# orm011/mplan2vdl

Measured on AMD Instinct MI355X. Metric: rows/s, TPC-H Q6 SF100 (fused VDL scan), + achieved HBM GB/s in roofline, higher is better.
Workload: dtype int64; 1 GPU; tpch_q6_sf100; rows_total=600037902, rows_per_gpu=600037902, bytes_per_row=28, finalise=local

## Files before the change

mplan2vdl_amd/csrc/vdl_jit.cpp:

```cpp
#include "vdl_jit.h"

#include <dlfcn.h>
#include <fcntl.h>
#include <sys/stat.h>
#include <unistd.h>

#include <atomic>
#include <cerrno>
#include <cstdio>
#include <cstdlib>
#include <cstring>
#include <fstream>
#include <map>
#include <mutex>
#include <sstream>

namespace vdl {
namespace jit {

namespace {

#ifndef VDL_PROJ_U
#define VDL_PROJ_U 4
#endif
// ... 223 lines not shown
        const MAggDesc &a = D.agg[j];
        o << "    d.agg[" << j << "].kind = " << a.kind << "; d.agg[" << j << "].used = " << a.used << "u; d.agg[" << j << "].plain = " << a.plain << "u; d.agg[" << j
          << "].constant = " << lit(a.constant) << ";\n";
        for (int k = 0; k < C.ncol; k++)
            if ((a.used >> k) & 1u) o << "    d.agg[" << j << "].fa[" << k << "] = " << lit(a.fa[k]) << "; d.agg[" << j << "].fs[" << k << "] = " << lit(a.fs[k]) << ";\n";
    }
    if (kind != MSCAN) {
        o << "    d.take = " << D.take << "u; d.nout = " << D.nout << "; d.bitmap_only = " << D.bitmap_only << "; d.carry = " << D.carry << "u;\n";
        for (int k = 0; k < D.nout; k++) o << "    d.out_col[" << k << "] = " << D.out_col[k] << ";\n";
        o << "    d.nexpr = " << D.nexpr << ";\n";
        for (int k = 0; k < D.nexpr; k++) o << "    d.expr_at[" << k << "] = " << D.expr_at[k] << "; d.expr_len[" << k << "] = " << D.expr_len[k] << ";\n";
    }
    o << "    return d;\n}\n}  // namespace vdl\n";
    return o.str();
}

static bool has_sat_diff(const MsArgs &C, const MScanDesc &D) {
    for (int k = 0; k < C.ncol; k++) if (D.dkind[k] == VC_SUBS) return true;
    return false;
}

static bool has_lookup_decode(const MsArgs &C) { return (C.decode & C.derived) != 0; }

std::string scan_source(Kind kind, const MsArgs &C, const MScanDesc &D, const Shape &sh) {
    std::ostringstream o;
    o << "#define VDL_SPEC_UNROLL _Pragma(\"unroll\")\n";
    const bool rt = sh.rt_bounds;
    if (rt) o << "#define VDL_RT_BOUNDS 1\n";
    if (has_sat_diff(C, D)) o << "#define VDL_SAT_DIFF 1\n";
    if (has_lookup_decode(C)) o << "#define VDL_LOOKUP_DECODE 1\n";
    if (kind == MSCAN && sh.batch) o << "#define VDL_BATCH " << sh.batch << "\n#define VDL_BATCH_NAGG " << D.nagg << "\n";
    if (kind == MSCAN && sh.census) o << "#define VDL_CENSUS 1\n";
    if (kind == MSCAN && C.packed) o << "#define VDL_PACKED 1\n";
    if (kind == MSCAN && C.lazy && C.packed) {
        auto ulit = [](int64_t x) { return std::to_string((uint64_t)x & 0xffffffffull) + "u"; };
        o << "#define VDL_STAGED_PRE";
        for (int c = 0; c < C.ncol; c++) {
            if (!((C.filtered >> c) & 1u) || ((C.lazy >> c) & 1u)) continue;
            if (rt) o << rt_filter_line(C, D, c, (C.packed >> c) & 1u);
            else if ((C.packed >> c) & 1u)
                o << " _Pragma(\"unroll\") for (int r = 0; r < RW; r++) alive[r] = alive[r] & ((uint32_t)v[" << c << "][r] >= " << ulit(D.flo[c]) << ") & ((uint32_t)v[" << c
                  << "][r] <= " << ulit(D.fhi[c]) << ");";
            else
                o << " _Pragma(\"unroll\") for (int r = 0; r < RW; r++) alive[r] = alive[r] & (v[" << c << "][r] >= " << lit(D.flo[c]) << ") & (v[" << c << "][r] <= "
                  << lit(D.fhi[c]) << ");";
        }
        o << "\n#define VDL_STAGED_POST";
        for (int c = 0; c < C.ncol; c++) {
            if (!((C.lazy >> c) & 1u)) continue;
            const int w = C.width(c);
            o << " { const __amdgpu_buffer_rsrc_t rs_ = buf_rsrc((const char *)Cr.ptr[" << c << "] + tile0 * " << w << ", (uint32_t)(tile_rows * " << w
              << ")); _Pragma(\"unroll\") for (int r = 0; r < RW; r++) {";
            if (sh.census)
                o << " { const uint64_t m_ = __ballot(pass[r]); const uint64_t a_ = (uint64_t)Cr.ptr[" << c << "] + (uint64_t)(rowid[r] - Cr.row0) * " << w << "ull;"
                  << " const int ln_ = (int)(threadIdx.x & 63u); int lo_ = ln_ - (int)((a_ & 127ull) / " << w << "ull); if (lo_ < 0) lo_ = 0;"
                  << " const bool first_ = pass[r] && ((m_ >> lo_) & ((1ull << (ln_ - lo_)) - 1ull)) == 0ull;"
                  << " const uint64_t f_ = __ballot(first_); if (ln_ == 0) census_cnt[" << c << "] += (unsigned long long)__popcll(f_); }";
            o << " v[" << c << "][r] = buf_load_one<" << w << ">(rs_, pass[r], (uint32_t)(rowid[r] - Cr.row0 - tile0) * " << w << "u); } }";
        }
        o << "\n";
    } else if (kind == MSCAN && C.lazy && C.queued) {
        o << "#define VDL_QUEUE_FILTER";
        for (int c = 0; c < C.ncol; c++)
            if (!((C.derived >> c) & 1u) && !((C.lazy >> c) & 1u) && ((C.filtered >> c) & 1u) && rt) o << rt_filter_line(C, D, c, false);
            else if (!((C.derived >> c) & 1u) && !((C.lazy >> c) & 1u) && ((C.filtered >> c) & 1u))
                o << " _Pragma(\"unroll\") for (int r = 0; r < RW; r++) alive[r] = alive[r] & (v[" << c << "][r] >= " << lit(D.flo[c]) << ") & (v[" << c << "][r] <= " << lit(D.fhi[c]) << ");";
// ... 24 lines not shown
                l << " if (RW % 2 == 0) { _Pragma(\"unroll\") for (int r = 0; r < RW; r += 2) { const int r1 = r + 1 < RW ? r + 1 : r; v[" << c << "][r] = 0; v[" << c
                  << "][r1] = 0;" << census(c, w, (std::string(mask) + "[r] | " + mask + "[r1]").c_str()) << " if (" << mask << "[r] | " << mask << "[r1]) { const int64_t i0 = rowid[r] - Cr.row0; if (i0 + 1 < Cr.n) { const " << vt << " x = *(const " << vt
                  << " *)((const char *)Cr.ptr[" << c << "] + i0 * " << w << "); v[" << c << "][r] = x.x; v[" << c << "][r1] = x.y; } else if (" << mask << "[r]) v[" << c
                  << "][r] = load_scalar(Cr.ptr[" << c << "], " << w << ", i0); } } } else {";
            }
            l << " _Pragma(\"unroll\") for (int r = 0; r < RW; r++) { v[" << c << "][r] = 0; if (" << mask << "[r]) v[" << c << "][r] = load_scalar(Cr.ptr[" << c << "], "
              << w << ", rowid[r] - Cr.row0); }";
            if (pairs) l << " }";
            return l.str();
        };
        o << "#define VDL_STAGED_PRE";
        for (int st = 0; st <= 3; st++)
            for (int c = 0; c < C.ncol; c++) {
                if (((C.derived >> c) & 1u) || C.stage(c) != st) continue;
                if (st > 0) o << load(c, "alive");
                if (((C.filtered >> c) & 1u) && rt) o << rt_filter_line(C, D, c, false);
                else if ((C.filtered >> c) & 1u)
                    o << " _Pragma(\"unroll\") for (int r = 0; r < RW; r++) alive[r] = alive[r] & (v[" << c << "][r] >= " << lit(D.flo[c]) << ") & (v[" << c << "][r] <= "
                      << lit(D.fhi[c]) << ");";
            }
        for (int c = 0; c < C.ncol; c++) if (!((C.derived >> c) & 1u) && C.stage(c) == 14) o << load(c, "alive");
        o << "\n#define VDL_STAGED_POST";
        for (int c = 0; c < C.ncol; c++) if (!((C.derived >> c) & 1u) && C.stage(c) == 15) o << load(c, "pass");
        o << "\n";
    }
    o << "#define VDL_PROJ_U " << VDL_PROJ_U_HOST << "\n" << kEmbedded << "\n" << desc_text(kind, C, D, "", rt);
    const char *b = sh.vec ? "true" : "false";
    if (kind == MSCAN && sh.batch)
        o << "extern \"C\" __global__ __launch_bounds__(256) void " << entry_name(kind, C, D, sh) << "(const vdl::MsArgs Cr, const vdl::MsBatch B) {\n"
             "    constexpr vdl::MsArgs C = vdl::jit_args();\n"
             "    constexpr vdl::MScanDesc D = vdl::jit_desc();\n"
             "    vdl::mscan_body<" << sh.nc << ", " << sh.u << ", " << b << ", " << b << ", " << (sh.grouped ? "true" : "false") << ", false, false>(C, Cr, D, *B.d[0], B);\n}\n";
    else if (kind == MSCAN)
        o << "extern \"C\" __global__ __launch_bounds__(256) void " << entry_name(kind, C, D, sh) << "(const vdl::MsArgs Cr, const vdl::MScanDesc *__restrict__ Dp) {\n"
             "    constexpr vdl::MsArgs C = vdl::jit_args();\n"
             "    constexpr vdl::MScanDesc D = vdl::jit_desc();\n"
             "    vdl::mscan_body<" << sh.nc << ", " << sh.u << ", " << b << ", " << b << ", " << (sh.grouped ? "true" : "false") << ", " << (sh.der ? "true" : "false")
          << ", " << (C.lazy ? "true" : "false") << ">(C, Cr, D, *Dp);\n}\n";
    else if (kind == SELECT)
        o << "extern \"C\" __global__ __launch_bounds__(256) void " << entry_name(kind) << "(const vdl::MsArgs Cr, const vdl::MScanDesc *__restrict__ Dp) {\n"
             "    constexpr vdl::MsArgs C = vdl::jit_args();\n"
             "    constexpr vdl::MScanDesc D = vdl::jit_desc();\n"
             "    vdl::project_select_body<" << sh.nc << ", vdl::kProjU, " << b << ", " << b << ">(C, Cr, D, *Dp);\n}\n";
    else
        o << "extern \"C\" __global__ __launch_bounds__(256) void " << entry_name(kind) << "(const vdl::MsArgs Cr, const vdl::MScanDesc *__restrict__ Dp, const uint16_t *__restrict__ scratch,\n"
             "        const int64_t *__restrict__ counts, const int64_t *__restrict__ offsets) {\n"
             "    constexpr vdl::MsArgs C = vdl::jit_args();\n"
             "    constexpr vdl::MScanDesc D = vdl::jit_desc();\n"
             "    vdl::project_take_body<" << sh.nc << ">(C, Cr, D, *Dp, scratch, counts, offsets);\n}\n";
    return o.str();
}
std::string mscan_source(const MsArgs &C, const MScanDesc &D, const Shape &sh) { return scan_source(MSCAN, C, D, sh); }
std::string front_source(const MsArgs &Cs, const MScanDesc &Ds, const MsArgs &Ct, const MScanDesc &Dt, const Shape &sh, int nct) {
    std::ostringstream o;
    o << "#define VDL_SPEC_UNROLL _Pragma(\"unroll\")\n";
    if (sh.rt_bounds) o << "#define VDL_RT_BOUNDS 1\n";
    if (has_sat_diff(Cs, Ds) || has_sat_diff(Ct, Dt)) o << "#define VDL_SAT_DIFF 1\n";
    if (has_lookup_decode(Cs) || has_lookup_decode(Ct)) o << "#define VDL_LOOKUP_DECODE 1\n";
    o << "#define VDL_PROJ_U " << VDL_PROJ_U_HOST << "\n#define VDL_FRONT_BATCH " << VDL_FRONT_BATCH_HOST << "\n" << kEmbedded << "\n" << desc_text(SELECT, Cs, Ds, "_s", sh.rt_bounds) << desc_text(TAKE, Ct, Dt, "_t", sh.rt_bounds);
    const char *b = sh.vec ? "true" : "false";
    o << "extern \"C\" __global__ __launch_bounds__(256) void " << entry_name(FRONT) << "(const vdl::MsArgs Csr, const vdl::MScanDesc *__restrict__ Dsp, const vdl::MsArgs Ctr,\n"
         "        const vdl::MScanDesc *__restrict__ Dtp, const vdl::FrontLook lk) {\n"
         "    constexpr vdl::MsArgs Cs = vdl::jit_args_s();\n"
         "    constexpr vdl::MScanDesc Ds = vdl::jit_desc_s();\n"
         "    constexpr vdl::MsArgs Ct = vdl::jit_args_t();\n"
         "    constexpr vdl::MScanDesc Dt = vdl::jit_desc_t();\n"
         "    vdl::project_front_body<" << sh.nc << ", " << nct << ", vdl::kProjU, " << b << ", " << b << ">(Cs, Csr, Ds, *Dsp, Ct, Ctr, Dt, *Dtp, lk);\n}\n";
    return o.str();
}
const char *entry_name(Kind kind) { return kind == MSCAN ? "vdl_jit_mscan" : kind == SELECT ? "vdl_jit_project_select" : kind == FRONT ? "vdl_jit_project_front" : "vdl_jit_project_take"; }
std::string entry_name(Kind kind, const MsArgs &C, const MScanDesc &D, const Shape &sh) {
    if (kind != MSCAN) return entry_name(kind);
    char tag[16];
    snprintf(tag, sizeof tag, "%06llx", (unsigned long long)(fnv(desc_text(kind, C, D, "", sh.rt_bounds)) & 0xffffffull));
    int eager_filters = 0;
    for (int c = 0; c < C.ncol; c++) eager_filters += ((C.filtered >> c) & 1u) && !((C.derived >> c) & 1u) && C.stage(c) == 0;
    return std::string("vdl_jit_mscan_") + (sh.grouped ? "grouped_" : "") + (C.packed ? "packed_" : "") + "u" + std::to_string(sh.u) + (C.lazy ? "_staged" + std::to_string(eager_filters) + "_" : "_") +
           (sh.census ? "census_" : "") + tag + (sh.batch ? "_batch" + std::to_string(sh.batch) : "") + (sh.rt_bounds ? "_rtb" : "");
}

bool compile(const std::string &src, const std::string &arch, std::vector<char> &code, std::string &log, Origin *origin) {
    if (origin) *origin = COMPILED;
    std::string key = std::to_string(fnv(src)) + "_" + std::to_string(src.size()) + "_" + arch;
    {
        Rtc &r0 = rtc();
        int major = 0, minor = 0;
        if (r0.lib && r0.version && r0.version(&major, &minor) == 0) key += "_rtc" + std::to_string(major) + "." + std::to_string(minor);
    }
    {
        std::lock_guard<std::mutex> g(g_mu);
        auto it = g_code.find(key);
        if (it != g_code.end()) { code = it->second; g_from_memory++; if (origin) *origin = FROM_MEMORY; return true; }
    }
    if (const char *dump = getenv("VDL_JIT_DUMP")) {
        std::ofstream f(std::string(dump) + "/vdl_" + key + ".hip");
        f << src;
    }
    const std::string dir = trusted_cache_dir();
    std::string path;
    if (!dir.empty()) {
        path = dir + "/vdl_" + key + ".vdlco";
        if (cache_read(path, src, code)) { std::lock_guard<std::mutex> g(g_mu); g_code[key] = code; g_from_disk++; if (origin) *origin = FROM_DISK; return true; }
    }
    Rtc &r = rtc();
    if (!r.lib || !r.why.empty()) { log = r.why.empty() ? "libhiprtc not usable" : r.why; return false; }
    void *prog = nullptr;
    if (r.create(&prog, src.c_str(), "vdl_jit_scan.hip", 0, nullptr, nullptr) != 0) { log = "hiprtcCreateProgram failed"; return false; }
    const std::string a = "--offload-arch=" + arch;
    const char *opts[] = {a.c_str(), "-O3", "-std=c++17"};
    const int rc = r.compile(prog, 3, opts);
// ... 30 lines not shown
```

mplan2vdl_amd/csrc/vdl_mscan_body.h:

```cpp
#pragma once
#include "vdl_scan_desc.h"
#include "vdl_front_index.h"

#ifndef VDL_SPEC_UNROLL
#define VDL_SPEC_UNROLL
#endif

namespace vdl {

typedef long long ll2 __attribute__((ext_vector_type(2)));
typedef int i32x2 __attribute__((ext_vector_type(2)));
typedef short i16x2 __attribute__((ext_vector_type(2)));
typedef char i8x2 __attribute__((ext_vector_type(2)));

template <int N> struct IntTag { static constexpr int value = N; };

namespace {


constexpr int kWave = 64;
constexpr int kMsBlock = 256;
#ifndef VDL_PROJ_U
#define VDL_PROJ_U 4
#endif
// ... 740 lines not shown
            int64_t t[RW];
            eval_term<NC, RW>(d, v, rowid, t);
            if (GROUPED) {
                if (rk == R_SUM) {
#pragma unroll
                    for (int r = 0; r < RW; r++) atomicAdd((unsigned long long *)&mytab[off[r] + 1 + j], (unsigned long long)t[r]);
                } else if (rk == R_MAX) {
#pragma unroll
                    for (int r = 0; r < RW; r++) atomicMax((long long *)&mytab[off[r] + 1 + j], (long long)t[r]);
                } else {
#pragma unroll
                    for (int r = 0; r < RW; r++) atomicMin((long long *)&mytab[off[r] + 1 + j], (long long)t[r]);
                }
            } else {
                int64_t s = r_identity(rk);
                if (rk == R_SUM) {
#pragma unroll
                    for (int r = 0; r < RW; r++) s = (int64_t)((uint64_t)s + (uint64_t)(pass[r] ? t[r] : 0));
                } else if (rk == R_MIN) {
#pragma unroll
                    for (int r = 0; r < RW; r++) s = (pass[r] && t[r] < s) ? t[r] : s;
                } else {
#pragma unroll
                    for (int r = 0; r < RW; r++) s = (pass[r] && t[r] > s) ? t[r] : s;
                }
                int64_t *slot = &lds[(int64_t)j * BS + tid];
                *slot = r_combine(rk, *slot, s);
            }
        }
    };

    const int64_t ntiles = Cr.n / TILE;
#ifdef VDL_PACKED
    if (!GROUPED && !DER && C.packed) {
        static_assert(32 % ROWS == 0, "a lane's 32 values of a stripe split into row slices");
        const int lane = tid & (kWave - 1);
        const int wave = __builtin_amdgcn_readfirstlane(tid / kWave);
        const int64_t nstripes = (Cr.n + 2047) / 2048, wstride = (int64_t)gridDim.x * (BS / kWave);
        for (int64_t s = (int64_t)blockIdx.x * (BS / kWave) + wave; s < nstripes; s += wstride) {
            uint32_t pw[NC][32];
#pragma unroll
            for (int c = 0; c < NC; c++) {
                if ((C.packed >> c) & 1u) {
                    const int b = C.bits(c);
                    const char *p = (const char *)Cr.ptr[c] + ((s * b) * kWave + lane) * 4;
#pragma unroll
                    for (int k = 0; k < 32; k++)
                        if (k < b) pw[c][k] = stream_load<NT, uint32_t>(p + (int64_t)k * (kWave * 4));
                }
            }
            __builtin_amdgcn_sched_barrier(0);
            const int64_t tile0 = s * 2048, tile_rows = Cr.n - tile0 < 2048 ? Cr.n - tile0 : 2048;
#pragma unroll
            for (int j0 = 0; j0 < 32; j0 += ROWS) {
                int64_t v[NC][ROWS], rowid[ROWS];
#pragma unroll
                for (int r = 0; r < ROWS; r++) rowid[r] = Cr.row0 + tile0 + (int64_t)(j0 + r) * kWave + lane;
#pragma unroll
                for (int c = 0; c < NC; c++) {
                    if ((C.packed >> c) & 1u) {
#pragma unroll
                        for (int r = 0; r < ROWS; r++) v[c][r] = (int64_t)unpack_bits(pw[c], j0 + r, C.bits(c));
                    } else if (c < C.ncol && !((C.lazy >> c) & 1u)) {
#pragma unroll
                        for (int r = 0; r < ROWS; r++) {
                            const int64_t i = rowid[r] - Cr.row0;
// ... 492 lines not shown
```

mplan2vdl_amd/csrc/vdl_scan_desc.h:

```cpp
#pragma once
#if defined(__HIPCC_RTC__)
typedef signed char int8_t;
typedef short int16_t;
typedef int int32_t;
typedef long long int64_t;
typedef unsigned char uint8_t;
typedef unsigned short uint16_t;
typedef unsigned int uint32_t;
typedef unsigned long long uint64_t;
typedef unsigned long long uintptr_t;
#define INT64_MAX 0x7fffffffffffffffLL
#define INT64_MIN (-INT64_MAX - 1)
#else
#include <cstdint>
#endif

#if defined(__HIPCC__) || defined(__HIPCC_RTC__)
#define VDL_SD __host__ __device__
#else
#define VDL_SD
#endif

namespace vdl {

// ... 88 lines not shown
    int64_t key_mask = 0;
    KeyComp comp[kMaxKeyComps];
    MAggDesc agg[kMaxGroupAggs];
    KeyStep key[kMaxKeySteps];
    unsigned long long *census = nullptr;
    uint32_t carry = 0;
    int64_t out_cap = INT64_MAX;
};
constexpr int kMaxCarry = 2;

constexpr int kMaxBatch = 8;
constexpr int kMaxBatchWords = 32;
constexpr int kMaxBatchGrouped = 4;
constexpr int kGroupLdsWords = 8192;
struct MsBatch {
    const MScanDesc *d[kMaxBatch] = {};
    int64_t *partials = nullptr;
};

struct MsArgs {
    int ncol = 0;
    uint32_t steps = 0;
    uint64_t widths = 0;
    uint32_t filtered = 0;
    uint32_t derived = 0;
    uint32_t lazy = 0;
    uint32_t decode = 0;
    uint64_t stages = 0;
    VDL_SD constexpr int stage(int c) const { return (int)((stages >> (4 * c)) & 15u); }
    int queued = 0;
    uint32_t packed = 0;
    uint64_t pbits = 0;
    VDL_SD constexpr int bits(int c) const { return c < 10 ? (int)((pbits >> (6 * c)) & 63u) : 0; }
    int64_t n = 0, row0 = 0;
    int64_t rowid_base = 0;
    const void *ptr[kMaxVCols] = {};
    VDL_SD constexpr int width(int c) const { return (int)((widths >> (4 * c)) & 15u); }
};

}
```

mplan2vdl_amd/csrc/vdl_scan_form.h:

```cpp
#pragma once
#include "vdl_scan_desc.h"

namespace vdl {

struct ScanForm {
    enum Kind { EAGER, STAGED, QUEUE, PACKED } kind = EAGER;
    static constexpr int kAllFilters = kMaxVCols;
    int eager_filters = 0;
    bool every_column = false;
    int u = 0;

    static ScanForm from_code(int code, int u = 0) {
        ScanForm f;
        f.u = u;
        f.kind = code <= 0 ? EAGER : code == 3 ? QUEUE : code >= 5 ? PACKED : STAGED;
        if (f.kind == STAGED) f.eager_filters = code == 4 ? kAllFilters : code;
        f.every_column = code >= 6;
        return f;
    }
    const char *suffix() const {
        return kind == EAGER ? "" : kind == QUEUE ? ",queue" : kind == PACKED ? (every_column ? ",packed" : ",packed,late")
             : eager_filters == kAllFilters ? ",lateall" : eager_filters > 1 ? ",late2" : ",late";
    }
};

}
```

mplan2vdl_amd/csrc/vdl_specialise.cpp:

```cpp
#include "vdl_specialise.h"

namespace vdl {
namespace eng {

void count_build(vdl_plan *p, const std::string &role, jit::Origin from) {
    std::pair<int, int> &b = p->jit_builds[role];
    b.first++;
    b.second += from != jit::COMPILED;
}
std::string builds_text(const vdl_plan *p, const std::string &role) {
    const auto it = p->jit_builds.find(role);
    if (it == p->jit_builds.end()) return "";
    return "from cache: " + std::to_string(it->second.second) + " of " + std::to_string(it->second.first) + " builds of " + role + "; ";
}

static jit::Shape jit_shape(const MScanCols &cols, const ScanLaunch &cfg, const ScanForm &f, bool rt) {
    jit::Shape sh;
    sh.rt_bounds = rt;
    mscan_variant_shape(cfg, &sh.nc, &sh.u, &sh.vec, &sh.grouped, &sh.der);
    sh.nc = cols.ncol;
    for (int k = 0; k < cols.ncol; k++) sh.der |= cols.kind[k] != VC_DIRECT;
    const char *u = getenv(sh.grouped ? "VDL_JIT_GROUP_U" : "VDL_JIT_U");
    if (u && atoi(u) >= 1 && atoi(u) <= 8) sh.u = atoi(u);
    if (f.u > 0) sh.u = f.u;
    else if (f.kind == ScanForm::PACKED) sh.u = getenv("VDL_JIT_U") ? atoi(getenv("VDL_JIT_U")) : 2;
    return sh;
}
static std::string jit_name(const jit::Shape &sh, const MScanCols &cols) {
    return "k_mscan_specialised<" + std::to_string(sh.nc) + "," + std::to_string(sh.u) + "," + (sh.vec ? "vec" : "novec") + "," + (sh.grouped ? "grouped" : "global") +
           (sh.der ? ",derived" : "") + (cols.image ? ",img" : "") + (cols.limage ? ",limg" : "") + ">";
}
static ScanForm form_asked_for() { return getenv("VDL_JIT_LATE") ? ScanForm::from_code(std::max(1, atoi(getenv("VDL_JIT_LATE")))) : ScanForm{}; }

static const std::vector<ScanColumn> &scan_columns(const vdl_plan *p, size_t s) {
    const size_t ns = p->fused.scans.size();
    return s < ns ? p->fused.scans[s].cols : p->fused.gscans[s - ns].cols;
}
static std::string short_name(const std::string &name) { return name.substr(name.find('.') == std::string::npos ? 0 : name.find('.') + 1); }
static std::string stages_text(const vdl_plan *p, size_t s, const MsArgs &args) {
    const std::vector<ScanColumn> &sc = scan_columns(p, s);
    std::string o;
    for (int k = 0; k < args.ncol && k < (int)sc.size(); k++) {
        const int st = args.stage(k);
        if (!st) continue;
        o += (o.empty() ? "" : " ") + short_name(sc[(size_t)k].name) + "@" + (st == 15 ? std::string("last") : st == 14 ? std::string("lookups") : std::to_string(st));
    }
    return o;
}
static std::string packed_text(const vdl_plan *p, size_t s, const MScanCols &cols) {
    const std::vector<ScanColumn> &sc = scan_columns(p, s);
    std::string o;
    for (int k = 0; k < cols.ncol && (size_t)k < sc.size(); k++)
        if ((cols.packed >> k) & 1u) o += (o.empty() ? "" : " ") + short_name(sc[(size_t)k].name) + ":" + std::to_string(cols.pbits[k]);
    return o;
}
static double sampled_selectivity(vdl_ctx *c, const void *dev, int width, int64_t n, int64_t lo, int64_t hi) {
    if (const char *a = getenv("VDL_JIT_ASSUME_SELECTIVITY")) return atof(a);
    if (n <= 0 || !dev || c->device < 0) return 1.0;
    const int64_t chunk = std::min<int64_t>(4096, n), pieces = std::max<int64_t>(1, std::min<int64_t>(16, n / chunk));
    std::vector<char> host((size_t)(chunk * width));
    int64_t in = 0, seen = 0;
    for (int64_t k = 0; k < pieces; k++) {
        const int64_t at = pieces > 1 ? (n - chunk) / (pieces - 1) * k : 0;
// ... 67 lines not shown
            }
            if (eager != 1) { why = "the queue form wants exactly one filter column with the tile"; return false; }
            args.queued = 1;
            args.stages = 0;
        }
        return true;
    }
    if (grouped || s >= p->fused.scans.size()) { why = "the packed form serves global aggregate scans only, not grouped scans"; return false; }
    const ScanPlan &sp = p->fused.scans[s];
    for (const ScanColumn &sc : sp.cols)
        if (sc.kind != VC_DIRECT) { why = "the packed form serves scans over table columns only, not scans with derived columns"; return false; }
    if (!c->images) { why = "column images are off"; return false; }
    if (u != 1 && u != 2 && u != 4 && u != 8 && u != 16) { why = "the packed form takes 1, 2, 4, 8 or 16 row pairs per slice (a lane's 32 values of a stripe split evenly)"; return false; }
    out.own_cols = std::make_shared<MScanCols>();
    out.own_desc = std::make_shared<MScanDesc>();
    MScanCols &pc = *out.own_cols;
    MScanDesc &pd = *out.own_desc;
    int64_t bpr = 0;
    bind_mscan(c, sp, pc, pd, &bpr, p->row_offset, f.every_column ? 2 : 1);
    pd.block_partials = d.block_partials;
    out.cols = &pc;
    out.desc = &pd;
    if (pc.ncol > 10) { why = "the packed form takes at most 10 columns"; return false; }
    if (!pc.packed) { why = f.every_column ? "no column has a packed image the scan may read" : "no filter column has a packed image the scan may read"; return false; }
    out.args = mscan_args(pc);
    if (!f.every_column) {
        MsArgs &args = out.args;
        uint32_t used = 0;
        for (int j = 0; j < pd.nagg; j++) if (pd.agg[j].kind != AGG_FIRST) used |= pd.agg[j].used;
        for (int k = 0; k < pc.ncol; k++)
            if (!((pc.packed >> k) & 1u) && !pc.filtered[k] && ((used >> k) & 1u)) { args.stages |= (uint64_t)15 << (4 * k); args.lazy |= 1u << k; }
        if (!args.lazy) { why = "no column to read late"; return false; }
    }
    return true;
}

struct Specialised {
    std::shared_ptr<jit::Kernel> k;
    int grid = 0, per_cu = 0;
    ScanForm form;
    size_t code_bytes = 0;
    std::string name, stages, packed;
    BoundForm b;
};
static bool build_specialised(vdl_ctx *c, vdl_plan *p, size_t s, bool grouped, const ScanForm &f, const MScanCols &cols, const MScanDesc &d, Specialised &out, std::string &why,
                              bool census = false) {
    out = Specialised{};
    jit::Shape sh = jit_shape(cols, p->mcfg[s], f, p->jit_rt_bounds);
    sh.census = census;
    std::vector<char> code;
    if (!bind_form(c, p, s, grouped, f, sh.u, cols, d, out.b, why)) return false;
    const MsArgs &args = out.b.args;
    const MScanDesc &desc = *out.b.desc;
    jit::Origin from = jit::COMPILED;
    if (!jit::compile(jit::mscan_source(args, desc, sh), c->arch, code, why, &from)) { why = why.substr(0, 400); return false; }
    count_build(p, "scan " + std::to_string(s), from);
    if (code.size() > (size_t)96 << 10) { why = "the descriptor did not fold (" + std::to_string(code.size()) + " B of code)"; return false; }
    out.k = jit::load(code, why, jit::entry_name(jit::MSCAN, args, desc, sh));
    if (!out.k) return false;
    int per_cu = 0;
    if (hipModuleOccupancyMaxActiveBlocksPerMultiprocessor(&per_cu, out.k->fn, 256, mscan_lds_bytes(desc, grouped)) != hipSuccess || per_cu < 1) {
        (void)hipGetLastError();
        per_cu = 2;
    }
    if (per_cu > 8) per_cu = 8;
    const int64_t tile = (int64_t)256 * 2 * sh.u;
    int64_t grid = (int64_t)c->num_cus * per_cu;
    const int64_t most = f.kind == ScanForm::PACKED ? (img::stripes(out.b.cols->n) + 3) / 4 : out.b.cols->n / tile;
    if (grid > most) grid = most;
    if (grid < 1) grid = 1;
    out.grid = (int)grid; out.per_cu = per_cu; out.code_bytes = code.size(); out.form = f; out.form.u = sh.u;
    out.name = jit_name(sh, *out.b.cols);
    out.name.insert(out.name.size() - 1, std::string(f.suffix()) + (sh.rt_bounds ? ",rtb" : ""));
    out.stages = stages_text(p, s, args);
    out.packed = packed_text(p, s, *out.b.cols);
    return true;
}
static std::string form_text(const Specialised &sp) {
    return (sp.packed.empty() ? "" : ", packed: " + sp.packed) + (sp.stages.empty() ? "" : ", read late: " + sp.stages);
}
static void install_form(vdl_plan *p, size_t s, const Specialised &sp) {
    int64_t *parts = p->mdesc[s].block_partials;
    p->mcols[s] = *sp.b.cols;
    p->mdesc[s] = *sp.b.desc;
    p->mdesc[s].block_partials = parts;
    p->mcfg[s].grid = sp.grid;
    p->mjit[s] = sp.k;
    p->mjit_form[s] = sp.form;
}
bool specialise_scan(vdl_ctx *c, vdl_plan *p, size_t s, bool grouped, std::string *kname) {
    Specialised sp;
    std::string why;
    const ScanForm late = form_asked_for();
    std::string why_late;
    if (late.kind != ScanForm::EAGER && !build_specialised(c, p, s, grouped, late, p->mcols[s], p->mdesc[s], sp, why_late) && late.kind == ScanForm::PACKED)
        p->jit_note += "scan " + std::to_string(s) + ": no packed form (" + why_late + "); ";
    if (!sp.k && !build_specialised(c, p, s, grouped, ScanForm{}, p->mcols[s], p->mdesc[s], sp, why)) { p->jit_note += "scan " + std::to_string(s) + ": not specialised (" + why + "); "; return false; }
    install_form(p, s, sp);
    *kname = sp.name;
    p->jit_note += "scan " + std::to_string(s) + ": " + sp.name + ", " + std::to_string(sp.code_bytes) + " B of code, " + std::to_string(sp.per_cu) + " blocks/CU" + form_text(sp) + "; " +
                   builds_text(p, "scan " + std::to_string(s));
    return true;
}

struct TimingEvents {
// ... 7 lines not shown
        HIP_CHECK(hipEventRecord(ev.a, c->stream));
        launch();
        HIP_CHECK(hipEventRecord(ev.b, c->stream));
        HIP_CHECK(hipEventSynchronize(ev.b));
        float t = 0;
        HIP_CHECK(hipEventElapsedTime(&t, ev.a, ev.b));
        if (rep > 0) times.push_back(t);
    }
    std::sort(times.begin(), times.end());
    return times[times.size() / 2];
}

void tune_specialised(vdl_ctx *c, vdl_plan *p, int64_t *dev_words) {
    const size_t ns = p->fused.scans.size(), ng = p->fused.gscans.size();
    TimingEvents ev;
    HIP_CHECK(hipEventCreate(&ev.a));
    HIP_CHECK(hipEventCreate(&ev.b));
    auto median_ms = [&](auto &&launch) { return median_launch_ms(c, ev, launch); };
    for (size_t s = 0; s < ns + ng; s++) {
        if (!p->mjit[s]) continue;
        const bool grouped = s >= ns;
        int64_t *out = dev_words + (grouped ? p->gword_offset[s - ns] : p->word_offset[s]);
        Specialised best;
        float best_ms = 0;
        std::string tried;
        std::vector<std::pair<int, int>> cands = {{2, 0}, {3, 0}, {4, 0}, {6, 0}, {0, 1}, {3, 1}, {2, 1}, {1, 1}, {3, 2}, {2, 2}, {4, 2}, {4, 3}, {3, 3}, {6, 3},
                                                  {2, 4}, {3, 4}, {4, 4}};
        int pin_u = 0, pin_late = -1;
        if (const char *pin = getenv("VDL_JIT_PIN")) {
            if (const char *q = strstr(pin, "u=")) pin_u = atoi(q + 2);
            if (const char *q = strstr(pin, "late=")) pin_late = atoi(q + 5);
            if (pin_u > 0) cands = {{pin_u, std::max(pin_late, 0)}};
        }
        std::vector<std::pair<int, int>> packed_forms = {{2, 5}, {4, 5}, {8, 5}, {16, 5}, {2, 6}, {4, 6}, {8, 6}};
        const char *packed_env = getenv("VDL_JIT_PACKED");
        if (pin_u > 0 || (packed_env && strcmp(packed_env, "0") == 0)) packed_forms.clear();
        else if (packed_env && strcmp(packed_env, "only") == 0) cands.clear();
        if (!packed_forms.empty()) {
            BoundForm b;
            std::string why;
            if (!bind_form(c, p, s, grouped, ScanForm::from_code(5), 2, p->mcols[s], p->mdesc[s], b, why) &&
                !bind_form(c, p, s, grouped, ScanForm::from_code(6), 2, p->mcols[s], p->mdesc[s], b, why)) packed_forms.clear();
        }
        cands.insert(cands.end(), packed_forms.begin(), packed_forms.end());
        const MScanCols *cols = &p->mcols[s];
        const MScanDesc *desc = &p->mdesc[s];
        MScanCols plain_cols;
        std::unique_ptr<MScanDesc> plain_desc;
        if (p->mjit_form[s].kind == ScanForm::PACKED) {
            plain_desc = std::make_unique<MScanDesc>();
            int64_t bpr = 0;
            bind_mscan(c, p->fused.scans[s], plain_cols, *plain_desc, &bpr, p->row_offset);
            plain_desc->block_partials = p->mdesc[s].block_partials;
            cols = &plain_cols;
            desc = plain_desc.get();
        }
        int best_u = 0;
        for (auto &cu : cands) {
            const ScanForm f = ScanForm::from_code(cu.second, cu.first ? cu.first : best_u);
            if (f.u <= 0 || (f.kind != ScanForm::PACKED && (int64_t)256 * 2 * f.u > cols->n)) continue;
            if (f.kind == ScanForm::STAGED && f.eager_filters == 1 && cu.first == best_u) continue;
            Specialised cand;
            std::string why;
            if (!build_specialised(c, p, s, grouped, f, *cols, *desc, cand, why)) continue;
            ScanLaunch cfg = p->mcfg[s];
            cfg.grid = cand.grid;
            HIP_CHECK(hipMemcpyAsync(p->mdev[s]->p, cand.b.desc, sizeof(MScanDesc), hipMemcpyHostToDevice, c->stream));
            const float ms = median_ms([&] { HIP_CHECK(launch_mscan(*cand.b.cols, *cand.b.desc, (const MScanDesc *)p->mdev[s]->p, cfg, grouped, false, out, false, c->stream, cand.k->fn)); });
            tried += " u=" + std::to_string(f.u) + f.suffix() + ":" + std::to_string((int)(ms * 1000)) + "us";
            if (!best.k || ms < best_ms * 0.98f) { best = cand; best_ms = ms; }
            if (f.kind == ScanForm::EAGER && (best_u == 0 || cand.k == best.k)) best_u = f.u;
        }
        if (!best.k) continue;
        if (!grouped && use_kscan(p->fused.scans[s]) && p->block_partials[s] && pin_u <= 0) {
            const float ms = median_ms([&] {
                HIP_CHECK(launch_scan(p->sargs[s], p->scfg[s], c->stream));
                HIP_CHECK(launch_scan_finish(p->sargs[s].block_partials, p->scfg[s].grid, p->sargs[s].nagg, nullptr, p->sargs[s], out, c->stream));
            });
            tried += std::string(" k_scan:") + std::to_string((int)(ms * 1000)) + "us";
            if (ms < best_ms * 0.98f) {
                p->kscan[s] = 1;
                p->mjit[s] = nullptr;
                p->jit_note += "scan " + std::to_string(s) + " tuned:" + tried + " -> " + scan_kernel_name(p->scfg[s]) + "; " + builds_text(p, "scan " + std::to_string(s));
                if ((int)s == p->dominant) p->dominant_kernel = std::string(scan_kernel_name(p->scfg[s])) + "_grid" + std::to_string(p->scfg[s].grid);
                continue;
            }
        }
        install_form(p, s, best);
        p->jit_note += "scan " + std::to_string(s) + " tuned:" + tried + " -> " + best.name + (best.packed.empty() ? "" : " (packed: " + best.packed + ")") +
                       (best.stages.empty() ? "" : " (read late: " + best.stages + ")") + "; " + builds_text(p, "scan " + std::to_string(s));
        if ((int)s == p->dominant)
            p->dominant_kernel = best.name + "_grid" + std::to_string(best.grid) + (grouped ? "_rep" + std::to_string(p->mdesc[s].replicas) : "");
    }
    p->description = describe_plan(p);
}

int64_t scan_bytes_moved(vdl_ctx *c, vdl_plan *p, std::string &detail) {
    if (!p->bound || p->dominant < 0) throw Error(VDL_ERR_ARG, "vdl_plan_scan_traffic: run the (fused) plan first");
    const size_t s = (size_t)p->dominant, ns = p->fused.scans.size();
    const bool grouped = s >= ns;
    const std::vector<ScanColumn> &sc = scan_columns(p, s);
    const bool staged = !(!grouped && p->kscan[s]) && p->mjit[s] && p->mjit_form[s].kind != ScanForm::EAGER;
// ... 39 lines not shown
                                                                               late ? "(late: " + std::to_string(lines[k]) + " lines of " + std::to_string((cols.n * cols.width[k] + 127) / 128) + ") " : " ");
    }
    detail += "(census of " + cen.name + (packed_form ? ")" : ", full tiles)");
    return total;
}

void jit_check_scans(vdl_ctx *c, vdl_plan *p) {
    if (!p->fused.ok) throw Error(VDL_ERR_UNSUPPORTED, "the plan has no fused scans: " + p->fused.why_not);
    const FusedPlan &F = p->fused;
    const size_t ns = F.scans.size();
    for (size_t s = 0; s < ns + F.gscans.size(); s++) {
        const bool grouped = s >= ns;
        MScanCols cols;
        auto d = std::make_unique<MScanDesc>();
        int64_t bpr = 0;
        if (grouped) bind_mscan(c, F.gscans[s - ns], cols, *d, &bpr, 0);
        else bind_mscan(c, F.scans[s], cols, *d, &bpr, 0);
        p->image_roles["scan" + std::to_string(s)] = image_text(scan_columns(p, s), cols);
        p->lookup_roles["scan" + std::to_string(s)] = lookup_text(scan_columns(p, s), cols);
        const ScanLaunch cfg = mscan_launch_config(cols, *d, grouped, c->num_cus);
        if (cfg.variant < 0) throw Error(VDL_ERR_UNSUPPORTED, "no scan kernel variant for this shape");
        const ScanForm late = form_asked_for();
        jit::Shape sh = jit_shape(cols, cfg, late, p->jit_rt_bounds);
        if (getenv("VDL_JIT_CENSUS")) sh.census = true;
        std::vector<char> code;
        std::string log;
        BoundForm b;
        if (!bind_form(c, p, s, grouped, late, sh.u, cols, *d, b, log)) {
            p->jit_note += "scan " + std::to_string(s) + ": not specialised (" + log + "); ";
            continue;
        }
        if (!jit::compile(jit::mscan_source(b.args, *b.desc, sh), c->arch, code, log))
            throw Error(VDL_ERR_UNSUPPORTED, "scan " + std::to_string(s) + " does not build: " + log.substr(0, 2000));
        std::string name = jit_name(sh, *b.cols);
        if (b.args.packed) name.insert(name.size() - 1, late.suffix());
        if (sh.rt_bounds) name.insert(name.size() - 1, ",rtb");
        p->jit_note += "scan " + std::to_string(s) + ": " + name + (b.args.packed ? " (packed: " + packed_text(p, s, *b.cols) + ")" : "") +
                       (b.args.queued ? " (queue)" : b.args.lazy ? " (late)" : "") + ", " + std::to_string(code.size()) + " B of code; ";
    }
}

std::string batch_alone_reason(const vdl_plan *p, bool grouped_on) {
    if (!p->use_fusion || !p->fused.ok) return "the plan is not fused";
    if (!p->use_jit) return "specialisation is off";
    const FusedPlan &F = p->fused;
    if (!F.gscans.empty() && !grouped_on) return "grouped scans are not batched";
    if (!F.gscans.empty()) {
        if (F.gscans.size() + F.scans.size() != 1) return "the plan has " + std::to_string(F.gscans.size() + F.scans.size()) + " scans, a batch shares exactly one";
        if (!F.prelude.empty()) return "scans with lookup tables or semi-join sets are not batched";
        for (const ScanColumn &sc : F.gscans[0].cols)
            if (sc.kind != VC_DIRECT) return "scans with derived columns are not batched";
        if (F.gscans[0].never) return "its filters can hold for no row: there is nothing to scan";
        return "";
    }
    if (F.scans.size() != 1) return "the plan has " + std::to_string(F.scans.size()) + " scans, a batch shares exactly one";
    if (!F.prelude.empty()) return "scans with lookup tables or semi-join sets are not batched";
    for (const ScanColumn &sc : F.scans[0].cols)
        if (sc.kind != VC_DIRECT) return "scans with derived columns are not batched";
    if (F.scans[0].never) return "its filters can hold for no row: there is nothing to scan";
    return "";
}
int batch_cap(int nagg) { return std::min(kMaxBatch, kMaxBatchWords / (1 + std::max(nagg, 0))); }
static int batch_width_asked() {
    const char *w = getenv("VDL_BATCH_WIDTH");
    return w && atoi(w) >= 2 ? atoi(w) : kMaxBatch;
}
int batch_cap_asked(int nagg) { return std::min(batch_cap(nagg), batch_width_asked()); }
// ... 202 lines not shown
```

Measured before the change: 1376 billion rows/s.

## Add packed scan form that prefetches next stripe while gathering late columns

Adds a new packed scan form (code 7, u=16) that double-buffers the packed bit-planes in registers. Each wave loads the next stripe before it evaluates aggregates on the current one, and issues the late-column gathers right after the filter mask is computed, so memory latency overlaps compute. The kernel gets a waves-per-EU hint, and the form is rejected if it would spill or exceed a register budget. The form joins the autotuned candidate list, so it only takes over when it times fastest; the cost is higher register pressure and lower occupancy.

```diff
diff --git a/mplan2vdl_amd/csrc/vdl_jit.cpp b/mplan2vdl_amd/csrc/vdl_jit.cpp
--- a/mplan2vdl_amd/csrc/vdl_jit.cpp
+++ b/mplan2vdl_amd/csrc/vdl_jit.cpp
@@ -279,6 +279,7 @@
     if (kind == MSCAN && sh.batch) o << "#define VDL_BATCH " << sh.batch << "\n#define VDL_BATCH_NAGG " << D.nagg << "\n";
     if (kind == MSCAN && sh.census) o << "#define VDL_CENSUS 1\n";
     if (kind == MSCAN && C.packed) o << "#define VDL_PACKED 1\n";
+    if (kind == MSCAN && C.packed && C.ahead()) o << "#define VDL_PACKED_AHEAD 1\n";
     if (kind == MSCAN && C.lazy && C.packed) {
         auto ulit = [](int64_t x) { return std::to_string((uint64_t)x & 0xffffffffull) + "u"; };
         o << "#define VDL_STAGED_PRE";
@@ -369,7 +370,7 @@
              "    constexpr vdl::MScanDesc D = vdl::jit_desc();\n"
              "    vdl::mscan_body<" << sh.nc << ", " << sh.u << ", " << b << ", " << b << ", " << (sh.grouped ? "true" : "false") << ", false, false>(C, Cr, D, *B.d[0], B);\n}\n";
     else if (kind == MSCAN)
-        o << "extern \"C\" __global__ __launch_bounds__(256) void " << entry_name(kind, C, D, sh) << "(const vdl::MsArgs Cr, const vdl::MScanDesc *__restrict__ Dp) {\n"
+        o << "extern \"C\" __global__ __launch_bounds__(256) " << (C.ahead() ? "__attribute__((amdgpu_waves_per_eu(3, 4))) " : "") << "void " << entry_name(kind, C, D, sh) << "(const vdl::MsArgs Cr, const vdl::MScanDesc *__restrict__ Dp) {\n"
              "    constexpr vdl::MsArgs C = vdl::jit_args();\n"
              "    constexpr vdl::MScanDesc D = vdl::jit_desc();\n"
              "    vdl::mscan_body<" << sh.nc << ", " << sh.u << ", " << b << ", " << b << ", " << (sh.grouped ? "true" : "false") << ", " << (sh.der ? "true" : "false")
@@ -412,7 +413,7 @@
     snprintf(tag, sizeof tag, "%06llx", (unsigned long long)(fnv(desc_text(kind, C, D, "", sh.rt_bounds)) & 0xffffffull));
     int eager_filters = 0;
     for (int c = 0; c < C.ncol; c++) eager_filters += ((C.filtered >> c) & 1u) && !((C.derived >> c) & 1u) && C.stage(c) == 0;
-    return std::string("vdl_jit_mscan_") + (sh.grouped ? "grouped_" : "") + (C.packed ? "packed_" : "") + "u" + std::to_string(sh.u) + (C.lazy ? "_staged" + std::to_string(eager_filters) + "_" : "_") +
+    return std::string("vdl_jit_mscan_") + (sh.grouped ? "grouped_" : "") + (C.packed ? "packed_" : "") + (C.ahead() ? "ahead_" : "") + "u" + std::to_string(sh.u) + (C.lazy ? "_staged" + std::to_string(eager_filters) + "_" : "_") +
            (sh.census ? "census_" : "") + tag + (sh.batch ? "_batch" + std::to_string(sh.batch) : "") + (sh.rt_bounds ? "_rtb" : "");
 }
 
diff --git a/mplan2vdl_amd/csrc/vdl_mscan_body.h b/mplan2vdl_amd/csrc/vdl_mscan_body.h
--- a/mplan2vdl_amd/csrc/vdl_mscan_body.h
+++ b/mplan2vdl_amd/csrc/vdl_mscan_body.h
@@ -796,6 +796,144 @@
 
     const int64_t ntiles = Cr.n / TILE;
 #ifdef VDL_PACKED
+#ifdef VDL_PACKED_AHEAD
+    if (!GROUPED && !DER && C.packed && C.ahead()) {
+        constexpr int RA = 4;
+        const int lane = tid & (kWave - 1);
+        const int wave = __builtin_amdgcn_readfirstlane(tid / kWave);
+        const int64_t nstripes = (Cr.n + 2047) / 2048, wstride = (int64_t)gridDim.x * (BS / kWave);
+        auto load_stripe = [&](int64_t st, uint32_t (&pw)[NC][32]) __attribute__((always_inline)) {
+            const bool there = st < nstripes;
+            int lane4 = lane * 4;
+            asm volatile("" : "+v"(lane4));
+#pragma unroll
+            for (int c = 0; c < NC; c++) {
+                if ((C.packed >> c) & 1u) {
+                    const int b = C.bits(c);
+                    const __amdgpu_buffer_rsrc_t rs = buf_rsrc((const char *)Cr.ptr[c] + (there ? st : 0) * (int64_t)(b * kWave * 4), there ? (uint32_t)(b * kWave * 4) : 0u);
+#pragma unroll
+                    for (int k = 0; k < 32; k++)
+                        if (k < b) pw[c][k] = __builtin_amdgcn_raw_buffer_load_b32(rs, lane4 + k * (kWave * 4), 0, NT ? 2 : 0);
+                }
+            }
+        };
+        int64_t racc[kMaxGroupAggs];
+#pragma unroll
+        for (int j = 0; j < kMaxGroupAggs; j++) racc[j] = j < nagg ? r_identity(rk_of(D.agg[j].kind)) : 0;
+        uint32_t used_by_terms = 0;
+#pragma unroll
+        for (int j = 0; j < kMaxGroupAggs; j++) if (j < nagg && D.agg[j].kind != AGG_FIRST) used_by_terms |= D.agg[j].used;
+        uint32_t pw_cur[NC][32], pw_next[NC][32];
+        int64_t s = (int64_t)blockIdx.x * (BS / kWave) + wave;
+        load_stripe(s, pw_cur);
+        for (; s < nstripes; s += wstride) {
+            const int64_t tile0 = s * 2048;
+            const int tile_rows = Cr.n - tile0 < 2048 ? (int)(Cr.n - tile0) : 2048;
+            uint32_t mask = 0;
+#pragma unroll
+            for (int j0 = 0; j0 < 32; j0 += RA) {
+                constexpr int RW = RA;
+                int64_t v[NC][RW];
+                bool alive[RW];
+#pragma unroll
+                for (int r = 0; r < RW; r++) alive[r] = (j0 + r) * kWave + lane < tile_rows;
+#pragma unroll
+                for (int c = 0; c < NC; c++) {
+#pragma unroll
+                    for (int r = 0; r < RW; r++) v[c][r] = ((C.packed & C.filtered) >> c) & 1u ? (int64_t)unpack_bits(pw_cur[c], j0 + r, C.bits(c)) : 0;
+                }
+                VDL_STAGED_PRE
+#pragma unroll
+                for (int r = 0; r < RW; r++) mask |= (uint32_t)alive[r] << (j0 + r);
+                __builtin_amdgcn_sched_barrier(0);
+            }
+            cnt += __popc(mask);
+            int32_t late[NC][32];
+#pragma unroll
+            for (int c = 0; c < NC; c++) {
+                if (c < C.ncol && ((C.lazy >> c) & 1u)) {
+                    const int w = C.width(c);
+                    const __amdgpu_buffer_rsrc_t rs = buf_rsrc((const char *)Cr.ptr[c] + tile0 * w, (uint32_t)(tile_rows * w));
+#pragma unroll
+                    for (int j = 0; j < 32; j++) {
+                        const bool on = (mask >> j) & 1u;
+                        const uint32_t off = (on ? (uint32_t)(lane * w) : kBufOut) + (uint32_t)(j * kWave * w);
+#ifdef VDL_CENSUS
+                        {
+                            const uint64_t m_ = __ballot(on);
+                            const uint64_t a_ = (uint64_t)Cr.ptr[c] + (uint64_t)(tile0 + j * kWave + lane) * (uint64_t)w;
+                            int lo_ = lane - (int)((a_ & 127ull) / (uint64_t)w);
+                            if (lo_ < 0) lo_ = 0;
+                            const bool first_ = on && ((m_ >> lo_) & ((1ull << (lane - lo_)) - 1ull)) == 0ull;
+                            const uint64_t f_ = __ballot(first_);
+                            if (lane == 0) census_cnt[c] += (unsigned long long)__popcll(f_);
+                        }
+#endif
+                        late[c][j] = w == 4 ? (int32_t)buf_load_one<4>(rs, true, off) : w == 2 ? (int32_t)buf_load_one<2>(rs, true, off) : (int32_t)buf_load_one<1>(rs, true, off);
+                    }
+                }
+            }
+            load_stripe(s + wstride, pw_next);
+            __builtin_amdgcn_sched_barrier(0);
+            uint32_t pw_again[NC][32];
+#pragma unroll
+            for (int c = 0; c < NC; c++) {
+#pragma unroll
+                for (int k = 0; k < 32; k++) {
+                    if (((C.packed & used_by_terms) >> c) & 1u && k < C.bits(c)) { pw_again[c][k] = pw_cur[c][k]; asm volatile("" : "+v"(pw_again[c][k])); }
+                    else pw_again[c][k] = 0;
+                }
+            }
+#pragma unroll
+            for (int j0 = 0; j0 < 32; j0 += RA) {
+                int64_t v[NC][RA], rowid[RA];
+                bool pass[RA];
+#pragma unroll
+                for (int r = 0; r < RA; r++) { rowid[r] = Cr.row0 + tile0 + (int64_t)((j0 + r) * kWave + lane); pass[r] = (mask >> (j0 + r)) & 1u; }
+#pragma unroll
+                for (int c = 0; c < NC; c++) {
+#pragma unroll
+                    for (int r = 0; r < RA; r++)
+                        v[c][r] = (C.packed >> c) & 1u ? (int64_t)unpack_bits(pw_again[c], j0 + r, C.bits(c)) : (c < C.ncol && ((C.lazy >> c) & 1u)) ? (int64_t)late[c][j0 + r] : 0;
+                }
+#pragma unroll
+                for (int j = 0; j < kMaxGroupAggs; j++) {
+                    if (j < nagg) {
+                        const int rk = rk_of(D.agg[j].kind);
+                        int64_t t[RA];
+                        eval_term<NC, RA>(D.agg[j], v, rowid, t);
+                        int64_t x = r_identity(rk);
+                        if (rk == R_SUM) {
+#pragma unroll
+                            for (int r = 0; r < RA; r++) x = (int64_t)((uint64_t)x + (uint64_t)(pass[r] ? t[r] : 0));
+                        } else if (rk == R_MIN) {
+#pragma unroll
+                            for (int r = 0; r < RA; r++) x = (pass[r] && t[r] < x) ? t[r] : x;
+                        } else {
+#pragma unroll
+                            for (int r = 0; r < RA; r++) x = (pass[r] && t[r] > x) ? t[r] : x;
+                        }
+                        racc[j] = r_combine(rk, racc[j], x);
+                    }
+                }
+                __builtin_amdgcn_sched_barrier(0);
+            }
+#pragma unroll
+            for (int c = 0; c < NC; c++) {
+#pragma unroll
+                for (int k = 0; k < 32; k++)
+                    if (((C.packed >> c) & 1u) && k < C.bits(c)) pw_cur[c][k] = pw_next[c][k];
+            }
+        }
+#pragma unroll
+        for (int j = 0; j < kMaxGroupAggs; j++) {
+            if (j < nagg) {
+                int64_t *slot = &lds[(int64_t)j * BS + tid];
+                *slot = r_combine(rk_of(D.agg[j].kind), *slot, racc[j]);
+            }
+        }
+    } else
+#endif
     if (!GROUPED && !DER && C.packed) {
         static_assert(32 % ROWS == 0, "a lane's 32 values of a stripe split into row slices");
         const int lane = tid & (kWave - 1);
diff --git a/mplan2vdl_amd/csrc/vdl_scan_desc.h b/mplan2vdl_amd/csrc/vdl_scan_desc.h
--- a/mplan2vdl_amd/csrc/vdl_scan_desc.h
+++ b/mplan2vdl_amd/csrc/vdl_scan_desc.h
@@ -144,6 +144,8 @@
     uint32_t packed = 0;
     uint64_t pbits = 0;
     VDL_SD constexpr int bits(int c) const { return c < 10 ? (int)((pbits >> (6 * c)) & 63u) : 0; }
+    static constexpr uint64_t kAheadBit = 1ull << 63;
+    VDL_SD constexpr bool ahead() const { return (pbits & kAheadBit) != 0; }
     int64_t n = 0, row0 = 0;
     int64_t rowid_base = 0;
     const void *ptr[kMaxVCols] = {};
diff --git a/mplan2vdl_amd/csrc/vdl_scan_form.h b/mplan2vdl_amd/csrc/vdl_scan_form.h
--- a/mplan2vdl_amd/csrc/vdl_scan_form.h
+++ b/mplan2vdl_amd/csrc/vdl_scan_form.h
@@ -1,5 +1,6 @@
 #pragma once
 #include "vdl_scan_desc.h"
+#include <string>
 
 namespace vdl {
 
@@ -8,6 +9,7 @@
     static constexpr int kAllFilters = kMaxVCols;
     int eager_filters = 0;
     bool every_column = false;
+    bool ahead = false;
     int u = 0;
 
     static ScanForm from_code(int code, int u = 0) {
@@ -15,13 +17,16 @@
         f.u = u;
         f.kind = code <= 0 ? EAGER : code == 3 ? QUEUE : code >= 5 ? PACKED : STAGED;
         if (f.kind == STAGED) f.eager_filters = code == 4 ? kAllFilters : code;
-        f.every_column = code >= 6;
+        f.every_column = code == 6;
+        f.ahead = code == 7;
         return f;
     }
     const char *suffix() const {
         return kind == EAGER ? "" : kind == QUEUE ? ",queue" : kind == PACKED ? (every_column ? ",packed" : ",packed,late")
              : eager_filters == kAllFilters ? ",lateall" : eager_filters > 1 ? ",late2" : ",late";
     }
+    const char *mark() const { return kind == PACKED && ahead ? ",ahead" : ""; }
+    std::string tried_suffix() const { return std::string(suffix()) + mark(); }
 };
 
 }
diff --git a/mplan2vdl_amd/csrc/vdl_specialise.cpp b/mplan2vdl_amd/csrc/vdl_specialise.cpp
--- a/mplan2vdl_amd/csrc/vdl_specialise.cpp
+++ b/mplan2vdl_amd/csrc/vdl_specialise.cpp
@@ -24,11 +24,12 @@
     if (u && atoi(u) >= 1 && atoi(u) <= 8) sh.u = atoi(u);
     if (f.u > 0) sh.u = f.u;
     else if (f.kind == ScanForm::PACKED) sh.u = getenv("VDL_JIT_U") ? atoi(getenv("VDL_JIT_U")) : 2;
+    if (f.kind == ScanForm::PACKED && f.ahead) sh.u = 16;
     return sh;
 }
-static std::string jit_name(const jit::Shape &sh, const MScanCols &cols) {
+static std::string jit_name(const jit::Shape &sh, const MScanCols &cols, const char *mark = "") {
     return "k_mscan_specialised<" + std::to_string(sh.nc) + "," + std::to_string(sh.u) + "," + (sh.vec ? "vec" : "novec") + "," + (sh.grouped ? "grouped" : "global") +
-           (sh.der ? ",derived" : "") + (cols.image ? ",img" : "") + (cols.limage ? ",limg" : "") + ">";
+           (sh.der ? ",derived" : "") + mark + (cols.image ? ",img" : "") + (cols.limage ? ",limg" : "") + ">";
 }
 static ScanForm form_asked_for() { return getenv("VDL_JIT_LATE") ? ScanForm::from_code(std::max(1, atoi(getenv("VDL_JIT_LATE")))) : ScanForm{}; }
 
@@ -162,6 +163,23 @@
             if (!((pc.packed >> k) & 1u) && !pc.filtered[k] && ((used >> k) & 1u)) { args.stages |= (uint64_t)15 << (4 * k); args.lazy |= 1u << k; }
         if (!args.lazy) { why = "no column to read late"; return false; }
     }
+    if (f.ahead) {
+        constexpr int kAheadRegisters = 96;
+        MsArgs &args = out.args;
+        int bits = 0, late_regs = 0;
+        for (int k = 0; k < pc.ncol; k++) {
+            if ((pc.packed >> k) & 1u) { bits += pc.pbits[k]; continue; }
+            if (!((args.lazy >> k) & 1u)) { why = "the form that reads ahead wants a packed image of every column it reads with the stripe"; return false; }
+            if (pc.width[k] > 4) { why = "the form that reads ahead keeps a late value in one register: no late column wider than 4 bytes"; return false; }
+            late_regs += 32;
+        }
+        if (2 * bits + late_regs > kAheadRegisters) {
+            why = "the form that reads ahead would keep " + std::to_string(2 * bits) + " packed dwords of two stripes and " + std::to_string(late_regs) +
+                  " late values per lane: more than " + std::to_string(kAheadRegisters) + " registers";
+            return false;
+        }
+        args.pbits |= MsArgs::kAheadBit;
+    }
     return true;
 }
 
@@ -188,6 +206,11 @@
     if (code.size() > (size_t)96 << 10) { why = "the descriptor did not fold (" + std::to_string(code.size()) + " B of code)"; return false; }
     out.k = jit::load(code, why, jit::entry_name(jit::MSCAN, args, desc, sh));
     if (!out.k) return false;
+    if (f.kind == ScanForm::PACKED && f.ahead) {
+        int scratch = 0;
+        if (hipFuncGetAttribute(&scratch, HIP_FUNC_ATTRIBUTE_LOCAL_SIZE_BYTES, out.k->fn) != hipSuccess) { (void)hipGetLastError(); scratch = 0; }
+        if (scratch > 0) { why = "the form that reads ahead spills (" + std::to_string(scratch) + " B of scratch memory per lane)"; return false; }
+    }
     int per_cu = 0;
     if (hipModuleOccupancyMaxActiveBlocksPerMultiprocessor(&per_cu, out.k->fn, 256, mscan_lds_bytes(desc, grouped)) != hipSuccess || per_cu < 1) {
         (void)hipGetLastError();
@@ -198,9 +221,10 @@
     int64_t grid = (int64_t)c->num_cus * per_cu;
     const int64_t most = f.kind == ScanForm::PACKED ? (img::stripes(out.b.cols->n) + 3) / 4 : out.b.cols->n / tile;
     if (grid > most) grid = most;
+    if (const char *g = getenv("VDL_JIT_GRID")) if (atoi(g) >= 1 && grid > atoi(g)) grid = atoi(g);
     if (grid < 1) grid = 1;
     out.grid = (int)grid; out.per_cu = per_cu; out.code_bytes = code.size(); out.form = f; out.form.u = sh.u;
-    out.name = jit_name(sh, *out.b.cols);
+    out.name = jit_name(sh, *out.b.cols, f.mark());
     out.name.insert(out.name.size() - 1, std::string(f.suffix()) + (sh.rt_bounds ? ",rtb" : ""));
     out.stages = stages_text(p, s, args);
     out.packed = packed_text(p, s, *out.b.cols);
@@ -274,7 +298,7 @@
             if (const char *q = strstr(pin, "late=")) pin_late = atoi(q + 5);
             if (pin_u > 0) cands = {{pin_u, std::max(pin_late, 0)}};
         }
-        std::vector<std::pair<int, int>> packed_forms = {{2, 5}, {4, 5}, {8, 5}, {16, 5}, {2, 6}, {4, 6}, {8, 6}};
+        std::vector<std::pair<int, int>> packed_forms = {{2, 5}, {4, 5}, {8, 5}, {16, 5}, {2, 6}, {4, 6}, {8, 6}, {16, 7}};
         const char *packed_env = getenv("VDL_JIT_PACKED");
         if (pin_u > 0 || (packed_env && strcmp(packed_env, "0") == 0)) packed_forms.clear();
         else if (packed_env && strcmp(packed_env, "only") == 0) cands.clear();
@@ -309,7 +333,7 @@
             cfg.grid = cand.grid;
             HIP_CHECK(hipMemcpyAsync(p->mdev[s]->p, cand.b.desc, sizeof(MScanDesc), hipMemcpyHostToDevice, c->stream));
             const float ms = median_ms([&] { HIP_CHECK(launch_mscan(*cand.b.cols, *cand.b.desc, (const MScanDesc *)p->mdev[s]->p, cfg, grouped, false, out, false, c->stream, cand.k->fn)); });
-            tried += " u=" + std::to_string(f.u) + f.suffix() + ":" + std::to_string((int)(ms * 1000)) + "us";
+            tried += " u=" + std::to_string(cand.form.u) + f.tried_suffix() + ":" + std::to_string((int)(ms * 1000)) + "us";
             if (!best.k || ms < best_ms * 0.98f) { best = cand; best_ms = ms; }
             if (f.kind == ScanForm::EAGER && (best_u == 0 || cand.k == best.k)) best_u = f.u;
         }
@@ -415,7 +439,7 @@
         }
         if (!jit::compile(jit::mscan_source(b.args, *b.desc, sh), c->arch, code, log))
             throw Error(VDL_ERR_UNSUPPORTED, "scan " + std::to_string(s) + " does not build: " + log.substr(0, 2000));
-        std::string name = jit_name(sh, *b.cols);
+        std::string name = jit_name(sh, *b.cols, b.args.ahead() ? late.mark() : "");
         if (b.args.packed) name.insert(name.size() - 1, late.suffix());
         if (sh.rt_bounds) name.insert(name.size() - 1, ",rtb");
         p->jit_note += "scan " + std::to_string(s) + ": " + name + (b.args.packed ? " (packed: " + packed_text(p, s, *b.cols) + ")" : "") +
```

After: 1282 billion rows/s. -6.8%, worse.
